# amcolex/ofdm-sync-math

Measured on AMD Instinct MI355X. Metric: complex Msamples/s through S&C metric kernel @ batch=65536; % HBM roofline, higher is better.
Workload: dtype f32 (c64 in, f64 prefix sums); 1 GPU; cfg3 Schmidl-Cox float32 metric+CFO, N=1024 (L=512), cir1, 65536 streams x 1024 c64 per GPU; global_batch=65536, seq_len=1024, L=512, parallelism=stream-shard x1 (no collectives), placement=auto -> contiguous

## Files before the change

ofdm-sync-math_amd/csrc/aa_fast.hip:

```cpp
#include <cfloat>
#include <cmath>
#include "ofs_common.h"
#include "aa_gate.h"
#include "ofdmsync.h"

using namespace ofs;

namespace {

constexpr int FAST_WG = 64;
constexpr int TMAX = 1024;
constexpr int FAST_CAP_LDS = 160 * 1024 / 10;
constexpr int FAST_CAP_LDS_FULL = 23000;

typedef float nf4 __attribute__((ext_vector_type(4)));
typedef float nf2 __attribute__((ext_vector_type(2)));
typedef float pf2 __attribute__((ext_vector_type(2)));
__device__ __forceinline__ pf2 mulc_acc(pf2 c, pf2 d, pf2 acc) {
    acc = __builtin_elementwise_fma(c, d.xx, acc);
    return __builtin_elementwise_fma(c.yx, pf2{d.y, -d.y}, acc);
}
template <int SP>
__device__ __forceinline__ void st_out(float4* p, float4 v) {
    const nf4 d = nf4{v.x, v.y, v.z, v.w};
    if constexpr (SP == 1) __builtin_nontemporal_store(d, reinterpret_cast<nf4*>(p));
    else *p = v;
}
template <int SP>
__device__ __forceinline__ void st_out(float2* p, float2 v) {
    const nf2 d = nf2{v.x, v.y};
    if constexpr (SP == 1) __builtin_nontemporal_store(d, reinterpret_cast<nf2*>(p));
    else *p = v;
}

template <int LP>
__device__ __forceinline__ float4 ld_x(const char* p) {
    if constexpr (LP == 1) {
        const nf4 v = __builtin_nontemporal_load(reinterpret_cast<const nf4*>(p));
        return make_float4(v.x, v.y, v.z, v.w);
    } else {
        return *reinterpret_cast<const float4*>(p);
    }
}

template <int SP>
__device__ __forceinline__ void st_rows2(float* span, const float (&a)[2], const float (&b)[2], int lane) {
    const bool odd = (lane & 1) != 0;
    const int idx = (lane < 32 ? 2 * lane : 2 * lane - 63) * 4;
    float o[4];
#pragma unroll
    for (int e = 0; e < 2; ++e) {
        const int ai = __float_as_int(a[e]), bi = __float_as_int(b[e]);
        const int bdn = dpp_i<0xA0>(bi);
        const int aup = dpp_i<0xF5>(ai);
        const int we = odd ? bdn : ai;
        const int wo = odd ? bi : aup;
        o[e] = __int_as_float(__builtin_amdgcn_ds_bpermute(idx, we));
        o[2 + e] = __int_as_float(__builtin_amdgcn_ds_bpermute(idx, wo));
    }
    st_out<SP>(reinterpret_cast<float4*>(span) + lane, make_float4(o[0], o[1], o[2], o[3]));
}


template <int E, int MR, int NA, bool DO, bool S32, int SV = 0, int FS = 0, int LP = 0>
__global__ __launch_bounds__(FAST_WG) void aa_fast_kernel(AaFastArgs a) {
    static_assert(SV == 0 || (E == 2 && NA == 1 && !DO), "store-path variants: one-antenna E = 2 storing kernel");
    static_assert(FS == 0 || (SV == 3 && !S32), "full-stream form: the headline's kernel");
    static_assert(LP == 0 || FS != 0, "load-policy arms: the full-stream form");
    constexpr bool FULL = FS != 0;
    constexpr int SP = SV & 1;
    constexpr bool RP = (SV & 2) != 0;
    constexpr int RL = 64 * E;
    constexpr int RW = TMAX / RL;
    constexpr int L = MR * RL;
    constexpr int V4 = E / 2;
    static_assert(MR >= 1 && MR <= RW, "window must fit the stream tile");
    const int lane = threadIdx.x & 63;
    const int w = FULL ? 0 : threadIdx.x >> 6;
    const int64_t b = (int64_t)(NA == 1 ? blockIdx.x : xcd_block()) + w;
    if (b >= a.B) return;
    const int T = FULL ? TMAX : (int)a.T;
    const uint32_t lo16 = 16u * (uint32_t)lane;
    float4 xreg[NA][RW][V4];
    if constexpr (FULL) {
        const char* const xb = reinterpret_cast<const char*>(a.x) + b * (TMAX * 8);
#pragma unroll
        for (int k = 0; k < RW; ++k) xreg[0][k][0] = ld_x<LP>(xb + RL * 8 * k + lo16);
    } else {
#pragma unroll
        for (int t = 0; t < NA; ++t) {
            const float2* xs = reinterpret_cast<const float2*>(a.x) + (b * NA + t) * a.T;
#pragma unroll
            for (int k = 0; k < RW; ++k)
#pragma unroll
                for (int j = 0; j < V4; ++j) {
                    int n = RL * k + E * lane + 2 * j;
                    n = n < T ? n : T - 2;
                    xreg[t][k][j] = *reinterpret_cast<const float4*>(xs + n);
                }
        }
    }
    auto xrow = [&](int t, int k, pf2 (&c)[E]) {
#pragma unroll
        for (int j = 0; j < V4; ++j) {
            const bool ok = FULL || RL * k + E * lane + 2 * j < T;
            const float4 v = xreg[t][k][j];
            c[2 * j] = ok ? pf2{v.x, v.y} : pf2{0.f, 0.f};
            c[2 * j + 1] = ok ? pf2{v.z, v.w} : pf2{0.f, 0.f};
        }
    };

    pf2 sS[MR][E];
    float sE[MR][E];
    double Cr[RW + 1], Ci[RW + 1], Ce[RW + 1];
    Cr[0] = Ci[0] = Ce[0] = 0.0;

    AaRowGate<E, float, false, (bool)(DO || NA == 1)> gate;
    const bool detect = FULL || a.detect;
    if (detect)
        gate.init(a.hyst, L, a.thr, a.fs, a.max_ev, a.ev_i + b * (int64_t)a.max_ev * 4,
                  a.ev_r + b * (int64_t)a.max_ev * 4);

    float* Pout = DO ? nullptr : reinterpret_cast<float*>(a.P);
    float* Rout = DO ? nullptr : reinterpret_cast<float*>(a.R);
    float* Mout = DO ? nullptr : reinterpret_cast<float*>(a.M);
    const float floor_ = 1e-6f * (float)L;
    float hR[2] = {0.f, 0.f}, hM[2] = {0.f, 0.f};
    const bool head = !DO && a.head_resident != 0;
    char* const Pb = FULL ? reinterpret_cast<char*>(a.P) + b * (TMAX * 8) : nullptr;
    float* const Rb = FULL ? reinterpret_cast<float*>(a.R) + b * TMAX : nullptr;
    float* const Mb = FULL ? reinterpret_cast<float*>(a.M) + b * TMAX : nullptr;

#pragma unroll
    for (int k = 0; k < RW; ++k) {
        if (FULL || RL * k < T) {
            const int nb = RL * k + E * lane;
            pf2 av[E];
            float aE[E];
#pragma unroll
            for (int e = 0; e < E; ++e) { av[e] = pf2{0.f, 0.f}; aE[e] = 0.f; }
#pragma unroll
            for (int t = 0; t < NA; ++t) {
                pf2 c[E];
                xrow(t, k, c);
// ... 302 lines not shown
        if (p < s.nrows) s.load_row(p, s.nx[p]);
    s.detect = a.detect != 0;
    if (s.detect)
        s.gate.init(a.hyst, S::L, a.thr, a.fs, a.max_ev, a.ev_i + b * (int64_t)a.max_ev * 4,
                    a.ev_r + b * (int64_t)a.max_ev * 4);
    s.Pout = DO ? nullptr : reinterpret_cast<float2*>(a.P);
    s.Rout = DO ? nullptr : reinterpret_cast<float*>(a.R);
    s.Mout = DO ? nullptr : reinterpret_cast<float*>(a.M);
    s.Vout = DO ? nullptr : a.valid;
    s.head = !DO && a.head_resident != 0;
    s.floor_ = 1e-6f * (float)S::L;

    s.template block<true, true>(0);
    int k0 = S::PER;
    for (; k0 + S::PER + S::PD <= s.full_rows; k0 += S::PER) s.template block<false, false>(k0);
    for (; k0 < s.nrows; k0 += S::PER) s.template block<false, true>(k0);
    if (a.detect) s.gate.finish(lane, s.Ti, a.n_ev + b);
}

template <int E, int MR, int NA>
int launch_stream(const AaFastArgs& a, hipStream_t st) {
    const bool det_only = a.detect && !a.P && !a.R && !a.M && !a.valid;
    constexpr int WGD = stream_wg(NA, true), WGS = stream_wg(NA, false);
    const int64_t grid = det_only ? (a.B + WGD / 64 - 1) / (WGD / 64) : (a.B + WGS / 64 - 1) / (WGS / 64);
    using S = AaStream<E, MR, NA, false>;
    constexpr size_t lag_lds = (size_t)(WGS / 64) * (S::LDSLAG ? MR : 1) * NA * S::V4 * 64 * 16;
    constexpr size_t cap_total = 24 * 1024;
    const size_t dflt = (!det_only && NA == 2 && cap_total > lag_lds) ? cap_total - lag_lds : 0;
    const size_t shm = ofs::variant(ofs::V_OCC_LDS) == INT64_MIN ? dflt : ofs::occ_lds();
    if (det_only)
        hipLaunchKernelGGL((aa_stream_kernel<E, MR, NA, true>), dim3((unsigned)grid), dim3(WGD), shm, st, a);
    else
        hipLaunchKernelGGL((aa_stream_kernel<E, MR, NA, false>), dim3((unsigned)grid), dim3(WGS), shm, st, a);
    return hipGetLastError() == hipSuccess ? 1 : OFS_EHIP;
}

template <int E, int NA>
int launch_stream_mr(int mr, const AaFastArgs& a, hipStream_t st) {
    if (mr == 8) return launch_stream<E, 8, NA>(a, st);
    if constexpr (E == 2) {
        switch (mr) {
            case 1: return launch_stream<E, 1, NA>(a, st);
            case 2: return launch_stream<E, 2, NA>(a, st);
            case 4: return launch_stream<E, 4, NA>(a, st);
        }
    }
    return 0;
}

bool scan32(bool det_only) {
    const int64_t v = ofs::variant(det_only ? ofs::V_FAST_SCAN_DO : ofs::V_FAST_SCAN);
    if (v == 32 || v == 64) return v == 32;
    return det_only;
}

float thr_as_f32(double thr) {
    if (thr != thr || thr == (double)INFINITY || thr == -(double)INFINITY) return (float)thr;
    if (thr > (double)FLT_MAX) return INFINITY;
    if (thr < -(double)FLT_MAX) return -FLT_MAX;
    float f = (float)thr;
    if ((double)f < thr) f = nextafterf(f, INFINITY);
    return f;
}

template <int E, int MR, int NA>
int launch(const AaFastArgs& a, hipStream_t st) {
    const bool det_only = a.detect && !a.P && !a.R && !a.M && !a.valid;
    const bool s32 = scan32(det_only);
    const dim3 grid((unsigned)a.B), blk(FAST_WG);
    const int64_t pad = ofs::variant_or(ofs::V_FAST_LDS, (!det_only && NA == 1) ? FAST_CAP_LDS : 0);
    const size_t shm = pad > 0 && pad <= 65536 ? (size_t)pad : 0;
    if constexpr (E == 2 && NA == 1) {
        if (!det_only && !s32) {
            const int sv = (ofs::variant_or(ofs::V_FAST_RMPAIR, 1) != 0 ? 2 : 0) | (ofs::variant_or(ofs::V_FAST_ST_POLICY, 1) == 1 ? 1 : 0);
            if constexpr (MR == 1 || MR == 2 || MR == 4) {
                if (sv == 3 && a.T == TMAX && a.P && a.R && a.M && !a.valid && a.detect && a.n_ev && a.ev_i && a.ev_r &&
                    !ofs::variant_off(ofs::V_FAST_FULL)) {
                    AaFastArgs f = a;
                    f.thr32 = thr_as_f32(a.thr);
                    const int64_t padf = ofs::variant_or(ofs::V_FAST_LDS, FAST_CAP_LDS_FULL);
                    const size_t shmf = padf > 0 && padf <= 65536 ? (size_t)padf : 0;
                    const bool ff = (a.hyst > 1 ? a.hyst : 1) >= 64 * E;
                    const bool nt = ofs::variant(ofs::V_FAST_LD_POLICY) != 0;
                    if (ff && nt) hipLaunchKernelGGL((aa_fast_kernel<E, MR, NA, false, false, 3, 1, 1>), grid, blk, shmf, st, f);
                    else if (ff) hipLaunchKernelGGL((aa_fast_kernel<E, MR, NA, false, false, 3, 1, 0>), grid, blk, shmf, st, f);
                    else if (nt) hipLaunchKernelGGL((aa_fast_kernel<E, MR, NA, false, false, 3, 2, 1>), grid, blk, shmf, st, f);
                    else hipLaunchKernelGGL((aa_fast_kernel<E, MR, NA, false, false, 3, 2, 0>), grid, blk, shmf, st, f);
                    return hipGetLastError() == hipSuccess ? 1 : OFS_EHIP;
                }
            }
            switch (sv) {
                case 0: hipLaunchKernelGGL((aa_fast_kernel<E, MR, NA, false, false, 0>), grid, blk, shm, st, a); break;
                case 1: hipLaunchKernelGGL((aa_fast_kernel<E, MR, NA, false, false, 1>), grid, blk, shm, st, a); break;
                case 2: hipLaunchKernelGGL((aa_fast_kernel<E, MR, NA, false, false, 2>), grid, blk, shm, st, a); break;
                default: hipLaunchKernelGGL((aa_fast_kernel<E, MR, NA, false, false, 3>), grid, blk, shm, st, a);
            }
            return hipGetLastError() == hipSuccess ? 1 : OFS_EHIP;
        }
    }
    if (det_only && s32) hipLaunchKernelGGL((aa_fast_kernel<E, MR, NA, true, true>), grid, blk, shm, st, a);
    else if (det_only) hipLaunchKernelGGL((aa_fast_kernel<E, MR, NA, true, false>), grid, blk, shm, st, a);
    else if (s32) hipLaunchKernelGGL((aa_fast_kernel<E, MR, NA, false, true>), grid, blk, shm, st, a);
    else hipLaunchKernelGGL((aa_fast_kernel<E, MR, NA, false, false>), grid, blk, shm, st, a);
    return hipGetLastError() == hipSuccess ? 1 : OFS_EHIP;
}

template <int E, int NA, int MR = 1>
int launch_mr(int mr, const AaFastArgs& a, hipStream_t st) {
    if constexpr (MR > TMAX / (64 * E)) {
        return 0;
    } else {
        if (mr == MR) return launch<E, MR, NA>(a, st);
        return launch_mr<E, NA, MR + 1>(mr, a, st);
    }
}

template <int NA>
int launch_e(int E, int mr, const AaFastArgs& a, hipStream_t st) {
    switch (E) {
        case 2: return launch_mr<2, NA>(mr, a, st);
        case 4: return launch_mr<4, NA>(mr, a, st);
        case 8: return launch_mr<8, NA>(mr, a, st);
    }
    return 0;
}

int pick_e(int L) {
    const int forced = (int)ofs::variant_or(ofs::V_FAST_E, 0);
    if (forced == 2 || forced == 4 || forced == 8) return (L % (64 * forced) == 0) ? forced : 0;
    for (int e : {2, 4, 8})
        if (L % (64 * e) == 0) return e;
    return 0;
}

int pick_e_do(int L) {
    const int forced = (int)ofs::variant_or(ofs::V_FAST_E_DO, 0);
    for (int e : {forced, 4, 8, 2})
        if ((e == 2 || e == 4 || e == 8) && L % (64 * e) == 0) return e;
    return 0;
}

}

int ofs_aa_fast_plan(int fmt, int precision, int n_ant, int64_t T, int L) {
    if (fmt != OFS_C64 || precision != OFS_FP32) return 0;
    if (n_ant != 1 && n_ant != 2) return 0;
    if (T < 1 || L < 128) return 0;
    if (T <= TMAX && !(T & 1) && L <= TMAX) {
        const int E = pick_e(L);
        if (E) return 10 * E + L / (64 * E);
    }
    if (T > 0x7fffffff - 1024) return 0;
    for (int e : {2, 4}) {
        if (L % (64 * e)) continue;
        const int mr = L / (64 * e);
        if (mr == 1 || mr == 2 || mr == 4 || mr == 8) return 100 + 10 * e + mr;
    }
    return 0;
}

int ofs_aa_fast_try(int fmt, int precision, int n_ant, const AaFastArgs& a, hipStream_t st) {
    const int plan = ofs_aa_fast_plan(fmt, precision, n_ant, a.T, a.L);
    if (!plan) return 0;
    if (plan >= 100) {
        const int E = (plan - 100) / 10, mr = plan % 10;
        if (E == 2) return n_ant == 1 ? launch_stream_mr<2, 1>(mr, a, st) : launch_stream_mr<2, 2>(mr, a, st);
// ... 10 lines not shown
```

ofdm-sync-math_amd/csrc/ofdmsync.hip:

```cpp
#include <hip/hip_runtime.h>
#include <stdint.h>
#include <math.h>
#include "ofdmsync.h"
#include "ofs_common.h"
#include <atomic>
#include <string.h>

namespace {

constexpr int WG = 256;
constexpr int EPT = 4;
constexpr int ROW = 64 * EPT;
constexpr int PASS = WG * EPT;
constexpr int EVBLK = 1024;
constexpr int MAXSLOT = 32;

enum Mode { M_AA = 0, M_SC = 1, M_COMB = 2, M_MINN = 3, M_RTL = 4 };

template <bool EX> struct Prec { using R = float; };
template <> struct Prec<true> { using R = double; };

template <int FMT, class R>
__device__ __forceinline__ void ldx(const void* p, int64_t i, R& re, R& im) {
    if constexpr (FMT == OFS_C64) {
// ... 644 lines not shown
    }
}

constexpr int LEN_MAX_FP32 = 3072;
constexpr int LEN_MAX_FP64 = 3584;

struct Plan { int64_t chunk; int32_t n_chunks, len_max, nrows_max; size_t lds; };

template <class R>
static int make_plan(int64_t T, int64_t n_out, int lo_x, int hi_x, int nq, bool exact, Plan& p) {
    const int halo = hi_x - lo_x;
    const int len_cap = exact ? LEN_MAX_FP64 : LEN_MAX_FP32;
    const int64_t chunk_cap = (int64_t)len_cap - halo;
    if (chunk_cap < 1) return OFS_ETOOLONG;
    int64_t n_chunks = (n_out + chunk_cap - 1) / chunk_cap;
    if (n_chunks < 1) n_chunks = 1;
    int64_t chunk = (n_out + n_chunks - 1) / n_chunks;
    int64_t max_len = chunk + halo;
    if (max_len > T) max_len = T;
    int len_max = (int)((max_len + 3) & ~3ll);
    if (len_max < 4) len_max = 4;
    const int nrows_max = ((len_max + PASS - 1) / PASS) * (PASS / ROW);
    p.chunk = chunk; p.n_chunks = (int32_t)n_chunks; p.len_max = len_max; p.nrows_max = nrows_max;
    p.lds = win_lds_bytes<R>(len_max, nrows_max, nq);
    return OFS_OK;
}

template <int FMT, bool EX, int MODE>
static int launch_win(WinArgs a, int64_t B, const Plan& p, hipStream_t st) {
    auto k = win_kernel<FMT, EX, MODE>;
    if (p.lds > 65536) {
        if (hipFuncSetAttribute((const void*)k, hipFuncAttributeMaxDynamicSharedMemorySize, (int)p.lds) != hipSuccess)
            return OFS_EHIP;
    }
    a.chunk = p.chunk; a.n_chunks = p.n_chunks; a.len_max = p.len_max; a.nrows_max = p.nrows_max;
    const int64_t grid = B * (int64_t)p.n_chunks;
    if (grid > 0x7fffffffll) return OFS_EINVAL;
    hipLaunchKernelGGL(k, dim3((unsigned)grid), dim3(WG), p.lds, st, a);
    return hipGetLastError() == hipSuccess ? OFS_OK : OFS_EHIP;
}

template <int MODE>
static int dispatch_win(int fmt, int precision, WinArgs a, int64_t B, int lo_x, int hi_x,
                        hipStream_t st, Plan* plan_out) {
    constexpr int nq = NQ<MODE>::v;
    Plan p;
    int rc;
    const bool ex = precision == OFS_FP64;
    rc = ex ? make_plan<double>(a.T, a.n_out, lo_x, hi_x, nq, true, p)
            : make_plan<float>(a.T, a.n_out, lo_x, hi_x, nq, false, p);
    if (rc) return rc;
    if (plan_out) *plan_out = p;
    a.lo_x = lo_x; a.hi_x = hi_x;
    if (ex) {
        switch (fmt) {
            case OFS_C64: return launch_win<OFS_C64, true, MODE>(a, B, p, st);
            case OFS_C128: return launch_win<OFS_C128, true, MODE>(a, B, p, st);
            case OFS_CI16: return launch_win<OFS_CI16, true, MODE>(a, B, p, st);
        }
    } else if constexpr (MODE != M_RTL) {
        switch (fmt) {
            case OFS_C64: return launch_win<OFS_C64, false, MODE>(a, B, p, st);
            case OFS_C128: return launch_win<OFS_C128, false, MODE>(a, B, p, st);
            case OFS_CI16: return launch_win<OFS_CI16, false, MODE>(a, B, p, st);
        }
    }
    return OFS_EINVAL;
}

static bool fmt_ok(int f) { return f == OFS_C64 || f == OFS_C128 || f == OFS_CI16; }
static bool prec_ok(int p) { return p == OFS_FP32 || p == OFS_FP64; }

}

extern "C" {

int32_t ofs_version(void) { return 100; }


static const char* const kVariantNames[ofs::V_COUNT] = {
    "EXACT", "FAST_E", "FAST_E_DO", "FAST_SCAN", "FAST_SCAN_DO", "RTL_WPB", "PARK_DIRECT", "ZW64",
    "ZW64_GRID", "ZS", "ZF_ITEMS", "ZS_PAIR", "ZS_DEFER", "ZS_BPL", "ZS_C", "ZS_GBLK", "MC_FUSED",
    "MC_FUSE_X", "ZC_SEQ", "ZC_NODMA", "BE_FAST", "MC_PERS", "FAST_LDS", "OCC_LDS",
    "FAST_RMPAIR", "FAST_ST_POLICY", "FAST_HEAD", "FAST_FULL", "FAST_LD_POLICY"};
struct VariantTable {
    int64_t v[ofs::V_COUNT];
    VariantTable() { for (auto& x : v) x = OFS_VARIANT_UNSET; }
};
static thread_local VariantTable g_variants;

static int variant_index(const char* name) {
    if (!name) return -1;
    for (int i = 0; i < ofs::V_COUNT; ++i)
        if (strcmp(name, kVariantNames[i]) == 0) return i;
    return -1;
}

int32_t ofs_debug_reset_variants(void) {
    for (auto& x : g_variants.v) x = OFS_VARIANT_UNSET;
    return OFS_OK;
}

int32_t ofs_debug_set_variant(const char* name, int64_t value) {
    const int i = variant_index(name);
    if (i < 0) return OFS_EINVAL;
    g_variants.v[i] = value;
    return OFS_OK;
}

int64_t ofs_debug_get_variant(const char* name) {
    const int i = variant_index(name);
    return i < 0 ? OFS_VARIANT_UNSET : ofs::variant((ofs::Variant)i);
}

const char* ofs_status_string(int32_t s) {
    switch (s) {
        case OFS_OK: return "ok";
        case OFS_EINVAL: return "invalid argument";
        case OFS_ETOOLONG: return "window/halo does not fit one LDS tile";
        case OFS_EHIP: return "HIP launch error";
        case OFS_ESHORT: return "stream shorter than one symbol";
        case OFS_EFFT: return "rocFFT error";
        default: return "unknown status";
    }
}

int32_t ofs_aa_detect(int32_t in_fmt, const void* x, int64_t B, int32_t n_ant, int64_t T,
                      int32_t L, int32_t precision, void* P, void* R, void* M, uint8_t* valid,
                      int32_t detect, double threshold, int32_t hysteresis, double sample_rate,
                      int32_t max_events, int32_t* n_events, int64_t* ev_int, double* ev_real,
                      void* stream) {
    return ofs_aa_detect_ex(in_fmt, x, B, n_ant, T, L, precision, P, R, M, valid, detect, threshold, hysteresis,
                            sample_rate, max_events, n_events, ev_int, ev_real, stream, 0u);
}

int32_t ofs_aa_detect_ex(int32_t in_fmt, const void* x, int64_t B, int32_t n_ant, int64_t T,
                         int32_t L, int32_t precision, void* P, void* R, void* M, uint8_t* valid,
                         int32_t detect, double threshold, int32_t hysteresis, double sample_rate,
                         int32_t max_events, int32_t* n_events, int64_t* ev_int, double* ev_real,
                         void* stream, uint32_t flags) {
    if (flags & ~(uint32_t)OFS_AA_HEAD_RESIDENT) return OFS_EINVAL;
    if (!(fmt_ok(in_fmt) || in_fmt == OFS_CP12) || !prec_ok(precision) || OFS_MISSING(x, B * T) || B < 0 || n_ant < 1 ||
        T < 0 || L < 1)
        return OFS_EINVAL;
    if (detect && (OFS_MISSING(n_events, B) || max_events < 0 ||
                   (max_events > 0 && B > 0 && (!ev_int || !ev_real))))
        return OFS_EINVAL;
    if (B == 0 || T == 0) return OFS_OK;
    hipStream_t st = (hipStream_t)stream;
    {
        AaFastArgs f{};
        f.x = x; f.B = B; f.T = T; f.L = L; f.P = P; f.R = R; f.M = M; f.valid = valid;
        f.detect = detect; f.thr = threshold; f.hyst = hysteresis; f.fs = sample_rate;
        f.max_ev = max_events; f.n_ev = n_events; f.ev_i = ev_int; f.ev_r = ev_real;
        f.head_resident = (flags & OFS_AA_HEAD_RESIDENT) != 0 && !ofs::variant_off(ofs::V_FAST_HEAD);
        int frc = ofs_aa_fast_try(in_fmt, precision, n_ant, f, st);
        if (frc == 1) return OFS_OK;
        if (frc < 0) return frc;
        frc = ofs_aa_exact_try(in_fmt, precision, n_ant, f, st);
        if (frc == 1) return OFS_OK;
        if (frc < 0) return frc;
    }
    if (in_fmt == OFS_CP12) return OFS_EINVAL;
    WinArgs a{};
    a.x = x; a.T = T; a.n_out = T; a.nb = n_ant; a.D = L; a.W = L;
    a.P = P; a.R = R; a.M = M; a.valid = valid;
    a.detect = detect; a.thr = threshold; a.hyst = hysteresis; a.fs = sample_rate;
// ... 205 lines not shown
```

ofdm-sync-math_amd/csrc/ofs_common.h:

```cpp
#pragma once
#include <hip/hip_runtime.h>
#include <stdint.h>

#define OFS_MISSING(p, n) ((p) == nullptr && (int64_t)(n) > 0)

namespace ofs {

enum Variant : int {
    V_EXACT, V_FAST_E, V_FAST_E_DO, V_FAST_SCAN, V_FAST_SCAN_DO, V_RTL_WPB, V_PARK_DIRECT, V_ZW64,
    V_ZW64_GRID, V_ZS, V_ZF_ITEMS, V_ZS_PAIR, V_ZS_DEFER, V_ZS_BPL, V_ZS_C, V_ZS_GBLK, V_MC_FUSED,
    V_MC_FUSE_X, V_ZC_SEQ, V_ZC_NODMA, V_BE_FAST, V_MC_PERS, V_FAST_LDS, V_OCC_LDS,
    V_FAST_RMPAIR, V_FAST_ST_POLICY, V_FAST_HEAD, V_FAST_FULL, V_FAST_LD_POLICY, V_COUNT
};
int64_t variant(Variant v);
inline bool variant_is(Variant v, int64_t value) { return variant(v) == value; }
inline bool variant_off(Variant v) { return variant(v) == 0; }
inline bool variant_on(Variant v) { const int64_t x = variant(v); return x != INT64_MIN && x != 0; }
inline int64_t variant_or(Variant v, int64_t dflt) { const int64_t x = variant(v); return x == INT64_MIN ? dflt : x; }
inline size_t occ_lds() { const int64_t x = variant(V_OCC_LDS); return x > 0 && x <= 65536 ? (size_t)x : 0; }


template <int CTRL>
__device__ __forceinline__ int dpp_i(int v) {
    return __builtin_amdgcn_mov_dpp(v, CTRL, 0xf, 0xf, false);
}
template <int CTRL>
__device__ __forceinline__ double dpp_d(double v) {
    const int lo = dpp_i<CTRL>(__double2loint(v));
    const int hi = dpp_i<CTRL>(__double2hiint(v));
    return __hiloint2double(hi, lo);
}

__device__ __forceinline__ double wave_scan_add(double v, int lane) {
    const int rl = lane & 15;
    double t;
    t = dpp_d<0x111>(v); if (rl >= 1) v += t;
    t = dpp_d<0x112>(v); if (rl >= 2) v += t;
    t = dpp_d<0x114>(v); if (rl >= 4) v += t;
    t = dpp_d<0x118>(v); if (rl >= 8) v += t;
    t = dpp_d<0x142>(v); if ((lane & 31) >= 16) v += t;
    t = dpp_d<0x143>(v); if (lane >= 32) v += t;
    return v;
}

__device__ __forceinline__ int wave_scan_max(int v, int lane) {
    const int rl = lane & 15;
    int t;
    t = dpp_i<0x111>(v); if (rl >= 1) v = max(v, t);
    t = dpp_i<0x112>(v); if (rl >= 2) v = max(v, t);
    t = dpp_i<0x114>(v); if (rl >= 4) v = max(v, t);
    t = dpp_i<0x118>(v); if (rl >= 8) v = max(v, t);
    t = dpp_i<0x142>(v); if ((lane & 31) >= 16) v = max(v, t);
    t = dpp_i<0x143>(v); if (lane >= 32) v = max(v, t);
    return v;
}

__device__ __forceinline__ double wave_shr1(double v, int lane, double first) {
    const double t = dpp_d<0x138>(v);
    return lane == 0 ? first : t;
}
__device__ __forceinline__ int wave_shr1(int v, int lane, int first) {
    const int t = dpp_i<0x138>(v);
    return lane == 0 ? first : t;
}

__device__ __forceinline__ double readlane(double v, int j) {
    const int lo = __builtin_amdgcn_readlane(__double2loint(v), j);
    const int hi = __builtin_amdgcn_readlane(__double2hiint(v), j);
    return __hiloint2double(hi, lo);
}
__device__ __forceinline__ float readlane(float v, int j) {
    return __int_as_float(__builtin_amdgcn_readlane(__float_as_int(v), j));
}
__device__ __forceinline__ int readlane(int v, int j) { return __builtin_amdgcn_readlane(v, j); }

template <int CTRL, int RMASK = 0xf>
__device__ __forceinline__ int dpp_old(int old, int v) {
    return __builtin_amdgcn_update_dpp(old, v, CTRL, RMASK, 0xf, false);
}
template <class Op>
__device__ __forceinline__ int dpp_reduce_bits(int v, int ident, Op op) {
    v = op(v, dpp_old<0x111>(ident, v));
    v = op(v, dpp_old<0x112>(ident, v));
    v = op(v, dpp_old<0x114>(ident, v));
    v = op(v, dpp_old<0x118>(ident, v));
    v = op(v, dpp_old<0x142, 0xa>(ident, v));
    v = op(v, dpp_old<0x143, 0xc>(ident, v));
    return __builtin_amdgcn_readlane(v, 63);
}
__device__ __forceinline__ float wave_max(float v) {
    const int r = dpp_reduce_bits(__float_as_int(v), __float_as_int(-__builtin_huge_valf()), [](int a, int b) {
        return __float_as_int(fmaxf(__int_as_float(a), __int_as_float(b)));
    });
    return __int_as_float(r);
}
// ... 32 lines not shown
    return blockIdx.x;
#endif
}

__device__ __forceinline__ float fast_atan2f(float y, float x) {
    const float ax = fabsf(x), ay = fabsf(y);
    const float mx = fmaxf(ax, ay), mn = fminf(ax, ay);
    const float a = mx > 0.f ? mn * __builtin_amdgcn_rcpf(mx) : 0.f;
    const float s = a * a;
    float r = -0.004054530523717403f;
    r = fmaf(r, s, 0.02186284027993679f);
    r = fmaf(r, s, -0.055912185460329056f);
    r = fmaf(r, s, 0.09642189741134644f);
    r = fmaf(r, s, -0.1390862762928009f);
    r = fmaf(r, s, 0.19946566224098206f);
    r = fmaf(r, s, -0.33329859375953674f);
    r = fmaf(r, s, 0.9999993443489075f);
    r *= a;
    if (ay > ax) r = 1.5707963267948966f - r;
    if (x < 0.f) r = 3.141592653589793f - r;
    return __builtin_copysignf(r, y);
}

template <int CTRL, int RMASK = 0xf>
__device__ __forceinline__ double dppz(double v) {
    const int lo = __builtin_amdgcn_update_dpp(0, __double2loint(v), CTRL, RMASK, 0xf, true);
    const int hi = __builtin_amdgcn_update_dpp(0, __double2hiint(v), CTRL, RMASK, 0xf, true);
    return __hiloint2double(hi, lo);
}
__device__ __forceinline__ double scan_add(double v) {
    v += dppz<0x111>(v);
    v += dppz<0x112>(v);
    v += dppz<0x114>(v);
    v += dppz<0x118>(v);
    v += dppz<0x142, 0xa>(v);
    v += dppz<0x143, 0xc>(v);
    return v;
}
__device__ __forceinline__ double shr1z(double v) { return dppz<0x138>(v); }

template <int CTRL, int RMASK = 0xf>
__device__ __forceinline__ int dppz_i(int v) {
    return __builtin_amdgcn_update_dpp(0, v, CTRL, RMASK, 0xf, true);
}
__device__ __forceinline__ int scan_add_i32(int v) {
    v += dppz_i<0x111>(v);
    v += dppz_i<0x112>(v);
    v += dppz_i<0x114>(v);
    v += dppz_i<0x118>(v);
    v += dppz_i<0x142, 0xa>(v);
    v += dppz_i<0x143, 0xc>(v);
    return v;
}

template <int CTRL, int RMASK = 0xf>
__device__ __forceinline__ float dppz_f(float v) {
    return __int_as_float(__builtin_amdgcn_update_dpp(0, __float_as_int(v), CTRL, RMASK, 0xf, true));
}
__device__ __forceinline__ float scan_add_f32(float v) {
    v += dppz_f<0x111>(v);
    v += dppz_f<0x112>(v);
    v += dppz_f<0x114>(v);
    v += dppz_f<0x118>(v);
    v += dppz_f<0x142, 0xa>(v);
    v += dppz_f<0x143, 0xc>(v);
    return v;
}

struct RowScan { float x, u; double tot; };
template <bool F32>
__device__ __forceinline__ RowScan row_scan(float v) {
    if constexpr (F32) {
        const float i = scan_add_f32(v);
        const float t = readlane(i, 63);
        return RowScan{dppz_f<0x138>(i), t - i, (double)t};
    } else {
        const double i = scan_add((double)v);
        const double t = readlane(i, 63);
        return RowScan{(float)shr1z(i), (float)(t - i), t};
    }
}


__device__ __forceinline__ void lds_dma16(const void* g, const void* lds) {
    const uint32_t m = (uint32_t)(uintptr_t)(__attribute__((address_space(3))) const void*)lds;
    asm volatile("s_mov_b32 m0, %1\n\ts_nop 0\n\tglobal_load_lds_dwordx4 %0, off" ::"v"(g), "s"(m) : "memory", "m0");
}


#define OFS_VMW(i) case i: asm volatile("s_waitcnt vmcnt(" #i ")" ::: "memory"); break;
__device__ __forceinline__ void vmcnt_wait(int n) {
    switch (n < 63 ? n : 63) {
        OFS_VMW(0) OFS_VMW(1) OFS_VMW(2) OFS_VMW(3) OFS_VMW(4) OFS_VMW(5) OFS_VMW(6) OFS_VMW(7)
        OFS_VMW(8) OFS_VMW(9) OFS_VMW(10) OFS_VMW(11) OFS_VMW(12) OFS_VMW(13) OFS_VMW(14) OFS_VMW(15)
        OFS_VMW(16) OFS_VMW(17) OFS_VMW(18) OFS_VMW(19) OFS_VMW(20) OFS_VMW(21) OFS_VMW(22) OFS_VMW(23)
        OFS_VMW(24) OFS_VMW(25) OFS_VMW(26) OFS_VMW(27) OFS_VMW(28) OFS_VMW(29) OFS_VMW(30) OFS_VMW(31)
        OFS_VMW(32) OFS_VMW(33) OFS_VMW(34) OFS_VMW(35) OFS_VMW(36) OFS_VMW(37) OFS_VMW(38) OFS_VMW(39)
        OFS_VMW(40) OFS_VMW(41) OFS_VMW(42) OFS_VMW(43) OFS_VMW(44) OFS_VMW(45) OFS_VMW(46) OFS_VMW(47)
        OFS_VMW(48) OFS_VMW(49) OFS_VMW(50) OFS_VMW(51) OFS_VMW(52) OFS_VMW(53) OFS_VMW(54) OFS_VMW(55)
        OFS_VMW(56) OFS_VMW(57) OFS_VMW(58) OFS_VMW(59) OFS_VMW(60) OFS_VMW(61) OFS_VMW(62)
        default: asm volatile("s_waitcnt vmcnt(63)" ::: "memory"); break;
    }
}
#undef OFS_VMW

}

struct AaFastArgs {
    const void* x;
    int64_t B, T;
    int32_t L;
    void* P; void* R; void* M; uint8_t* valid;
    int32_t detect; double thr; int32_t hyst; double fs;
    int32_t max_ev; int32_t* n_ev; int64_t* ev_i; double* ev_r;
    int32_t head_resident;
    float thr32;
};
int ofs_aa_fast_try(int fmt, int precision, int n_ant, const AaFastArgs& a, hipStream_t st);
int ofs_aa_fast_plan(int fmt, int precision, int n_ant, int64_t T, int L);

int ofs_aa_exact_plan(int fmt, int precision, int n_ant, int64_t T, int L);
int ofs_aa_exact_try(int fmt, int precision, int n_ant, const AaFastArgs& a, hipStream_t st);
struct RtlExactCall {
    const void* x; int64_t B, T; int32_t Q;
    int32_t shift, smooth_mode, frac_bits; double thr_value;
    double* corr_total; double* corr_positive; double* smooth; double* energy_total;
    double* corr_scaled; double* energy_scaled; uint8_t* mvalid; uint8_t* above;
    int32_t detect, hyst, toff, max_ev; int32_t* n_ev; int64_t* ev; int64_t* open_start;
};
int ofs_rtl_exact_plan(int fmt, int n_br, int64_t T, int Q);
int ofs_rtl_exact_try(int fmt, int n_br, const RtlExactCall& c, hipStream_t st);

struct WinFastArgs {
    const void* x; int64_t B, T; int N;
    void* M; void* P; void* R;
};
int ofs_win_fast_try(int mode, int fmt, int precision, int n_br, const WinFastArgs& a, hipStream_t st);
int ofs_win_fast_plan(int mode, int fmt, int precision, int n_br, int64_t T, int N);
int ofs_sc_minn_fast_plan(int fmt, int precision, int n_br, int64_t T, int N);
int ofs_sc_minn_fast_try(int fmt, int precision, int n_br, const void* x, int64_t B, int64_t T, int N,
                         void* Ms, void* Ps, void* Rs, void* Mm, void* Pm, void* Rm, hipStream_t st);
```

Measured before the change: 359,800 Msamples/s.

## Add lean full-stream Schmidl-Cox kernel with register-resident input and batched DPP scans

Adds a specialised one-antenna, full-stream metric kernel that loads the whole 1024-sample stream into registers up front, interleaves three row scans (energy, real and imaginary correlation) with DPP row broadcasts that keep their registers, and delays R/M stores by one row pair. It becomes the default path for the headline configuration unless FAST_LEAN is turned off. The aim is to cut instruction count and scan latency relative to the general templated kernel and to hide load latency by issuing every load early. In exchange it uses more VGPRs for the register tile and carries a second copy of the kernel logic that has to stay in sync with the original.

```diff
diff --git a/ofdm-sync-math_amd/csrc/aa_fast.hip b/ofdm-sync-math_amd/csrc/aa_fast.hip
--- a/ofdm-sync-math_amd/csrc/aa_fast.hip
+++ b/ofdm-sync-math_amd/csrc/aa_fast.hip
@@ -2,64 +2,17 @@
 #include <cmath>
 #include "ofs_common.h"
 #include "aa_gate.h"
+#include "aa_fast_io.h"
 #include "ofdmsync.h"
 
 using namespace ofs;
 
+int ofs_aa_lean_launch(int mr, bool ff, bool nt, bool head, unsigned grid, size_t shm, hipStream_t st, const AaFastArgs& f);
+
 namespace {
 
-constexpr int FAST_WG = 64;
-constexpr int TMAX = 1024;
 constexpr int FAST_CAP_LDS = 160 * 1024 / 10;
 constexpr int FAST_CAP_LDS_FULL = 23000;
-
-typedef float nf4 __attribute__((ext_vector_type(4)));
-typedef float nf2 __attribute__((ext_vector_type(2)));
-typedef float pf2 __attribute__((ext_vector_type(2)));
-__device__ __forceinline__ pf2 mulc_acc(pf2 c, pf2 d, pf2 acc) {
-    acc = __builtin_elementwise_fma(c, d.xx, acc);
-    return __builtin_elementwise_fma(c.yx, pf2{d.y, -d.y}, acc);
-}
-template <int SP>
-__device__ __forceinline__ void st_out(float4* p, float4 v) {
-    const nf4 d = nf4{v.x, v.y, v.z, v.w};
-    if constexpr (SP == 1) __builtin_nontemporal_store(d, reinterpret_cast<nf4*>(p));
-    else *p = v;
-}
-template <int SP>
-__device__ __forceinline__ void st_out(float2* p, float2 v) {
-    const nf2 d = nf2{v.x, v.y};
-    if constexpr (SP == 1) __builtin_nontemporal_store(d, reinterpret_cast<nf2*>(p));
-    else *p = v;
-}
-
-template <int LP>
-__device__ __forceinline__ float4 ld_x(const char* p) {
-    if constexpr (LP == 1) {
-        const nf4 v = __builtin_nontemporal_load(reinterpret_cast<const nf4*>(p));
-        return make_float4(v.x, v.y, v.z, v.w);
-    } else {
-        return *reinterpret_cast<const float4*>(p);
-    }
-}
-
-template <int SP>
-__device__ __forceinline__ void st_rows2(float* span, const float (&a)[2], const float (&b)[2], int lane) {
-    const bool odd = (lane & 1) != 0;
-    const int idx = (lane < 32 ? 2 * lane : 2 * lane - 63) * 4;
-    float o[4];
-#pragma unroll
-    for (int e = 0; e < 2; ++e) {
-        const int ai = __float_as_int(a[e]), bi = __float_as_int(b[e]);
-        const int bdn = dpp_i<0xA0>(bi);
-        const int aup = dpp_i<0xF5>(ai);
-        const int we = odd ? bdn : ai;
-        const int wo = odd ? bi : aup;
-        o[e] = __int_as_float(__builtin_amdgcn_ds_bpermute(idx, we));
-        o[2 + e] = __int_as_float(__builtin_amdgcn_ds_bpermute(idx, wo));
-    }
-    st_out<SP>(reinterpret_cast<float4*>(span) + lane, make_float4(o[0], o[1], o[2], o[3]));
-}
 
 
 template <int E, int MR, int NA, bool DO, bool S32, int SV = 0, int FS = 0, int LP = 0>
@@ -528,6 +481,8 @@
                     const size_t shmf = padf > 0 && padf <= 65536 ? (size_t)padf : 0;
                     const bool ff = (a.hyst > 1 ? a.hyst : 1) >= 64 * E;
                     const bool nt = ofs::variant(ofs::V_FAST_LD_POLICY) != 0;
+                    if (!ofs::variant_off(ofs::V_FAST_LEAN))
+                        return ofs_aa_lean_launch(MR, ff, nt, a.head_resident != 0, (unsigned)a.B, shmf, st, f);
                     if (ff && nt) hipLaunchKernelGGL((aa_fast_kernel<E, MR, NA, false, false, 3, 1, 1>), grid, blk, shmf, st, f);
                     else if (ff) hipLaunchKernelGGL((aa_fast_kernel<E, MR, NA, false, false, 3, 1, 0>), grid, blk, shmf, st, f);
                     else if (nt) hipLaunchKernelGGL((aa_fast_kernel<E, MR, NA, false, false, 3, 2, 1>), grid, blk, shmf, st, f);
diff --git a/ofdm-sync-math_amd/csrc/aa_fast_io.h b/ofdm-sync-math_amd/csrc/aa_fast_io.h
--- /dev/null
+++ b/ofdm-sync-math_amd/csrc/aa_fast_io.h
@@ -0,0 +1,57 @@
+#pragma once
+#include "ofs_common.h"
+
+namespace {
+using ofs::dpp_i;
+
+constexpr int FAST_WG = 64;
+constexpr int TMAX = 1024;
+typedef float nf4 __attribute__((ext_vector_type(4)));
+typedef float nf2 __attribute__((ext_vector_type(2)));
+typedef float pf2 __attribute__((ext_vector_type(2)));
+__device__ __forceinline__ pf2 mulc_acc(pf2 c, pf2 d, pf2 acc) {
+    acc = __builtin_elementwise_fma(c, d.xx, acc);
+    return __builtin_elementwise_fma(c.yx, pf2{d.y, -d.y}, acc);
+}
+template <int SP>
+__device__ __forceinline__ void st_out(float4* p, float4 v) {
+    const nf4 d = nf4{v.x, v.y, v.z, v.w};
+    if constexpr (SP == 1) __builtin_nontemporal_store(d, reinterpret_cast<nf4*>(p));
+    else *p = v;
+}
+template <int SP>
+__device__ __forceinline__ void st_out(float2* p, float2 v) {
+    const nf2 d = nf2{v.x, v.y};
+    if constexpr (SP == 1) __builtin_nontemporal_store(d, reinterpret_cast<nf2*>(p));
+    else *p = v;
+}
+
+template <int LP>
+__device__ __forceinline__ float4 ld_x(const char* p) {
+    if constexpr (LP == 1) {
+        const nf4 v = __builtin_nontemporal_load(reinterpret_cast<const nf4*>(p));
+        return make_float4(v.x, v.y, v.z, v.w);
+    } else {
+        return *reinterpret_cast<const float4*>(p);
+    }
+}
+
+template <int SP>
+__device__ __forceinline__ void st_rows2(float* span, const float (&a)[2], const float (&b)[2], int lane) {
+    const bool odd = (lane & 1) != 0;
+    const int idx = (lane < 32 ? 2 * lane : 2 * lane - 63) * 4;
+    float o[4];
+#pragma unroll
+    for (int e = 0; e < 2; ++e) {
+        const int ai = __float_as_int(a[e]), bi = __float_as_int(b[e]);
+        const int bdn = dpp_i<0xA0>(bi);
+        const int aup = dpp_i<0xF5>(ai);
+        const int we = odd ? bdn : ai;
+        const int wo = odd ? bi : aup;
+        o[e] = __int_as_float(__builtin_amdgcn_ds_bpermute(idx, we));
+        o[2 + e] = __int_as_float(__builtin_amdgcn_ds_bpermute(idx, wo));
+    }
+    st_out<SP>(reinterpret_cast<float4*>(span) + lane, make_float4(o[0], o[1], o[2], o[3]));
+}
+
+}
diff --git a/ofdm-sync-math_amd/csrc/aa_lean.hip b/ofdm-sync-math_amd/csrc/aa_lean.hip
--- /dev/null
+++ b/ofdm-sync-math_amd/csrc/aa_lean.hip
@@ -0,0 +1,176 @@
+#include "ofs_common.h"
+#include "aa_gate.h"
+#include "aa_fast_io.h"
+#include "ofdmsync.h"
+
+using namespace ofs;
+
+namespace {
+
+__device__ __forceinline__ float4 shuf_rows2(const float (&a)[2], const float (&b)[2], int lane) {
+    const bool odd = (lane & 1) != 0;
+    const int idx = (lane < 32 ? 2 * lane : 2 * lane - 63) * 4;
+    float o[4];
+#pragma unroll
+    for (int e = 0; e < 2; ++e) {
+        const int ai = __float_as_int(a[e]), bi = __float_as_int(b[e]);
+        const int bdn = dpp_i<0xA0>(bi);
+        const int aup = dpp_i<0xF5>(ai);
+        const int we = odd ? bdn : ai;
+        const int wo = odd ? bi : aup;
+        o[e] = __int_as_float(__builtin_amdgcn_ds_bpermute(idx, we));
+        o[2 + e] = __int_as_float(__builtin_amdgcn_ds_bpermute(idx, wo));
+    }
+    return make_float4(o[0], o[1], o[2], o[3]);
+}
+
+template <int MR, int FS, int LP, bool HD>
+__global__ __launch_bounds__(FAST_WG) void aa_lean_kernel(AaFastArgs a) {
+    constexpr int E = 2, SP = 1;
+    constexpr int RL = 64 * E;
+    constexpr int RW = TMAX / RL;
+    constexpr int L = MR * RL;
+    static_assert(MR >= 1 && MR <= RW - 2, "the last row pair lies behind the window");
+    const int lane = threadIdx.x & 63;
+    const int64_t b = (int64_t)blockIdx.x;
+    if (b >= a.B) return;
+    constexpr int T = TMAX;
+    const uint32_t lo16 = 16u * (uint32_t)lane;
+    float4 xreg[RW];
+    const char* const xb = reinterpret_cast<const char*>(a.x) + b * (TMAX * 8);
+#pragma unroll
+    for (int k = 0; k < RW; ++k) xreg[k] = ld_x<LP>(xb + RL * 8 * k + lo16);
+    auto xrow = [&](int k, pf2 (&c)[E]) {
+        const float4 v = xreg[k];
+        c[0] = pf2{v.x, v.y};
+        c[1] = pf2{v.z, v.w};
+    };
+
+    pf2 sS[MR][E];
+    float sE[MR][E];
+    double Cr[RW + 1], Ci[RW + 1], Ce[RW + 1];
+    Cr[0] = Ci[0] = Ce[0] = 0.0;
+
+    AaRowGate<E, float, false, true> gate;
+    gate.init(a.hyst, L, a.thr, a.fs, a.max_ev, a.ev_i + b * (int64_t)a.max_ev * 4, a.ev_r + b * (int64_t)a.max_ev * 4);
+
+    const float floor_ = 1e-6f * (float)L;
+    float hR[2] = {0.f, 0.f}, hM[2] = {0.f, 0.f};
+    constexpr bool head = HD;
+    ScanKeep zk[3];
+    float4 oR = make_float4(0.f, 0.f, 0.f, 0.f), oM = oR;
+    char* const Pb = reinterpret_cast<char*>(a.P) + b * (TMAX * 8);
+    float* const Rb = reinterpret_cast<float*>(a.R) + b * TMAX;
+    float* const Mb = reinterpret_cast<float*>(a.M) + b * TMAX;
+
+#pragma unroll
+    for (int k = 0; k < RW; ++k) {
+        const int nb = RL * k + E * lane;
+        pf2 av[E];
+        float aE[E];
+#pragma unroll
+        for (int e = 0; e < E; ++e) { av[e] = pf2{0.f, 0.f}; aE[e] = 0.f; }
+        {
+            pf2 c[E];
+            xrow(k, c);
+#pragma unroll
+            for (int e = 0; e < E; ++e) aE[e] += fmaf(c[e].x, c[e].x, c[e].y * c[e].y);
+            if (k >= MR) {
+                pf2 d[E];
+                xrow(k - MR, d);
+#pragma unroll
+                for (int e = 0; e < E; ++e) av[e] = mulc_acc(c[e], d[e], av[e]);
+            }
+        }
+        pf2 fS[E], gS[E];
+        float fE[E], gE[E];
+        fS[0] = av[0]; fE[0] = aE[0];
+#pragma unroll
+        for (int e = 1; e < E; ++e) { fS[e] = fS[e - 1] + av[e]; fE[e] = fE[e - 1] + aE[e]; }
+        gS[E - 1] = pf2{0.f, 0.f}; gE[E - 1] = 0.f;
+#pragma unroll
+        for (int e = E - 2; e >= 0; --e) { gS[e] = gS[e + 1] + av[e + 1]; gE[e] = gE[e + 1] + aE[e + 1]; }
+        RowScan sEr, sRr{0.f, 0.f, 0.0}, sIr{0.f, 0.f, 0.0};
+        if (k >= MR) {
+            const float v3[3] = {fE[E - 1], fS[E - 1].x, fS[E - 1].y};
+            RowScan r3[3];
+            row_scan_keep3(v3, zk, r3);
+            sEr = r3[0]; sRr = r3[1]; sIr = r3[2];
+        } else {
+            sEr = row_scan_keep(fE[E - 1], zk[0]);
+        }
+        if (k >= 2 && (k & 1) == 0) {
+            st_out<SP>(reinterpret_cast<float4*>(Rb + RL * (k - 2)) + lane, oR);
+            if (!(k - 1 < MR && head)) st_out<SP>(reinterpret_cast<float4*>(Mb + RL * (k - 2)) + lane, oM);
+        }
+        const double totR = sRr.tot, totI = sIr.tot, totE = sEr.tot;
+        const pf2 xS = pf2{sRr.x, sIr.x};
+        const float xE = sEr.x;
+        const pf2 uS = pf2{sRr.u, sIr.u};
+        const float uE = sEr.u;
+        Cr[k + 1] = Cr[k] + totR; Ci[k + 1] = Ci[k] + totI; Ce[k + 1] = Ce[k] + totE;
+        const pf2 wS = pf2{(float)((k >= MR) ? (Cr[k] - Cr[k - MR + 1]) : Cr[k]),
+                           (float)((k >= MR) ? (Ci[k] - Ci[k - MR + 1]) : Ci[k])};
+        const float wE = (float)((k >= MR) ? (Ce[k] - Ce[k - MR + 1]) : Ce[k]);
+
+        float pf[E][2], mf[E], pmf[E], rf[E];
+#pragma unroll
+        for (int e = 0; e < E; ++e) {
+            pf2 P = wS + (xS + fS[e]);
+            float RR = wE + (xE + fE[e]);
+            if (k >= MR) { P += sS[k % MR][e]; RR += sE[k % MR][e]; }
+            sS[k % MR][e] = uS + gS[e]; sE[k % MR][e] = uE + gE[e];
+            const float pm = fmaf(P.x, P.x, P.y * P.y);
+            float m = 0.f;
+            if (k >= MR && RR > floor_) m = fminf(pm * __builtin_amdgcn_rcpf(RR * RR), 1.f);
+            pf[e][0] = P.x; pf[e][1] = P.y; rf[e] = RR; mf[e] = m; pmf[e] = pm;
+        }
+
+        const bool pm_row = !(k < MR && head);
+        if (pm_row) st_out<SP>(reinterpret_cast<float4*>(Pb + RL * 8 * k + lo16), make_float4(pf[0][0], pf[0][1], pf[1][0], pf[1][1]));
+        if ((k & 1) == 0) {
+            hR[0] = rf[0]; hR[1] = rf[1]; hM[0] = mf[0]; hM[1] = mf[1];
+        } else {
+            oR = shuf_rows2(hR, rf, lane);
+            if (pm_row) oM = shuf_rows2(hM, mf, lane);
+        }
+
+        if (k >= MR) {
+            float pr[E], pi[E];
+#pragma unroll
+            for (int e = 0; e < E; ++e) { pr[e] = pf[e][0]; pi[e] = pf[e][1]; }
+            bool ab[E];
+#pragma unroll
+            for (int e = 0; e < E; ++e) ab[e] = mf[e] >= a.thr32;
+            gate.template row_flags<FS, true>(lane, k, nb, T, ab, pmf, pr, pi, mf);
+        }
+    }
+    st_out<SP>(reinterpret_cast<float4*>(Rb + RL * (RW - 2)) + lane, oR);
+    st_out<SP>(reinterpret_cast<float4*>(Mb + RL * (RW - 2)) + lane, oM);
+    gate.finish(lane, T, a.n_ev + b);
+}
+
+template <int MR>
+int launch_lean(bool ff, bool nt, bool head, dim3 grid, dim3 blk, size_t shm, hipStream_t st, const AaFastArgs& f) {
+#define OFS_LEAN(FS_, LP_) \
+    do { if (head) hipLaunchKernelGGL((aa_lean_kernel<MR, FS_, LP_, true>), grid, blk, shm, st, f); \
+         else hipLaunchKernelGGL((aa_lean_kernel<MR, FS_, LP_, false>), grid, blk, shm, st, f); } while (0)
+    if (ff && nt) OFS_LEAN(1, 1);
+    else if (ff) OFS_LEAN(1, 0);
+    else if (nt) OFS_LEAN(2, 1);
+    else OFS_LEAN(2, 0);
+#undef OFS_LEAN
+    return hipGetLastError() == hipSuccess ? 1 : OFS_EHIP;
+}
+
+}
+
+int ofs_aa_lean_launch(int mr, bool ff, bool nt, bool head, unsigned grid, size_t shm, hipStream_t st, const AaFastArgs& f) {
+    const dim3 g(grid), blk(FAST_WG);
+    switch (mr) {
+        case 1: return launch_lean<1>(ff, nt, head, g, blk, shm, st, f);
+        case 2: return launch_lean<2>(ff, nt, head, g, blk, shm, st, f);
+        case 4: return launch_lean<4>(ff, nt, head, g, blk, shm, st, f);
+    }
+    return 0;
+}
diff --git a/ofdm-sync-math_amd/csrc/ofdmsync.hip b/ofdm-sync-math_amd/csrc/ofdmsync.hip
--- a/ofdm-sync-math_amd/csrc/ofdmsync.hip
+++ b/ofdm-sync-math_amd/csrc/ofdmsync.hip
@@ -750,7 +750,7 @@
     "EXACT", "FAST_E", "FAST_E_DO", "FAST_SCAN", "FAST_SCAN_DO", "RTL_WPB", "PARK_DIRECT", "ZW64",
     "ZW64_GRID", "ZS", "ZF_ITEMS", "ZS_PAIR", "ZS_DEFER", "ZS_BPL", "ZS_C", "ZS_GBLK", "MC_FUSED",
     "MC_FUSE_X", "ZC_SEQ", "ZC_NODMA", "BE_FAST", "MC_PERS", "FAST_LDS", "OCC_LDS",
-    "FAST_RMPAIR", "FAST_ST_POLICY", "FAST_HEAD", "FAST_FULL", "FAST_LD_POLICY"};
+    "FAST_RMPAIR", "FAST_ST_POLICY", "FAST_HEAD", "FAST_FULL", "FAST_LD_POLICY", "FAST_LEAN"};
 struct VariantTable {
     int64_t v[ofs::V_COUNT];
     VariantTable() { for (auto& x : v) x = OFS_VARIANT_UNSET; }
diff --git a/ofdm-sync-math_amd/csrc/ofs_common.h b/ofdm-sync-math_amd/csrc/ofs_common.h
--- a/ofdm-sync-math_amd/csrc/ofs_common.h
+++ b/ofdm-sync-math_amd/csrc/ofs_common.h
@@ -10,7 +10,7 @@
     V_EXACT, V_FAST_E, V_FAST_E_DO, V_FAST_SCAN, V_FAST_SCAN_DO, V_RTL_WPB, V_PARK_DIRECT, V_ZW64,
     V_ZW64_GRID, V_ZS, V_ZF_ITEMS, V_ZS_PAIR, V_ZS_DEFER, V_ZS_BPL, V_ZS_C, V_ZS_GBLK, V_MC_FUSED,
     V_MC_FUSE_X, V_ZC_SEQ, V_ZC_NODMA, V_BE_FAST, V_MC_PERS, V_FAST_LDS, V_OCC_LDS,
-    V_FAST_RMPAIR, V_FAST_ST_POLICY, V_FAST_HEAD, V_FAST_FULL, V_FAST_LD_POLICY, V_COUNT
+    V_FAST_RMPAIR, V_FAST_ST_POLICY, V_FAST_HEAD, V_FAST_FULL, V_FAST_LD_POLICY, V_FAST_LEAN, V_COUNT
 };
 int64_t variant(Variant v);
 inline bool variant_is(Variant v, int64_t value) { return variant(v) == value; }
@@ -209,6 +209,56 @@
 }
 
 
+struct ScanKeep { int l15 = 0, h15 = 0, l31 = 0, h31 = 0; };
+template <int CTRL, int RMASK>
+__device__ __forceinline__ double dpp_keep(double v, int& lo, int& hi) {
+    lo = __builtin_amdgcn_update_dpp(lo, __double2loint(v), CTRL, RMASK, 0xf, true);
+    hi = __builtin_amdgcn_update_dpp(hi, __double2hiint(v), CTRL, RMASK, 0xf, true);
+    return __hiloint2double(hi, lo);
+}
+__device__ __forceinline__ RowScan row_scan_keep(float v, ScanKeep& z) {
+    double i = (double)v;
+    i += dppz<0x111>(i);
+    i += dppz<0x112>(i);
+    i += dppz<0x114>(i);
+    i += dppz<0x118>(i);
+    i += dpp_keep<0x142, 0xa>(i, z.l15, z.h15);
+    i += dpp_keep<0x143, 0xc>(i, z.l31, z.h31);
+    const double t = readlane(i, 63);
+    return RowScan{dppz_f<0x138>((float)i), (float)(t - i), t};
+}
+template <int CTRL>
+__device__ __forceinline__ void scan_step3(double (&i)[3]) {
+    double t[3];
+#pragma unroll
+    for (int j = 0; j < 3; ++j) t[j] = dppz<CTRL>(i[j]);
+#pragma unroll
+    for (int j = 0; j < 3; ++j) i[j] += t[j];
+}
+__device__ __forceinline__ void row_scan_keep3(const float (&v)[3], ScanKeep (&z)[3], RowScan (&r)[3]) {
+    double i[3], t[3];
+#pragma unroll
+    for (int j = 0; j < 3; ++j) i[j] = (double)v[j];
+    scan_step3<0x111>(i);
+    scan_step3<0x112>(i);
+    scan_step3<0x114>(i);
+    scan_step3<0x118>(i);
+#pragma unroll
+    for (int j = 0; j < 3; ++j) t[j] = dpp_keep<0x142, 0xa>(i[j], z[j].l15, z[j].h15);
+#pragma unroll
+    for (int j = 0; j < 3; ++j) i[j] += t[j];
+#pragma unroll
+    for (int j = 0; j < 3; ++j) t[j] = dpp_keep<0x143, 0xc>(i[j], z[j].l31, z[j].h31);
+#pragma unroll
+    for (int j = 0; j < 3; ++j) i[j] += t[j];
+#pragma unroll
+    for (int j = 0; j < 3; ++j) {
+        const double tot = readlane(i[j], 63);
+        r[j] = RowScan{dppz_f<0x138>((float)i[j]), (float)(tot - i[j]), tot};
+    }
+}
+
+
 __device__ __forceinline__ void lds_dma16(const void* g, const void* lds) {
     const uint32_t m = (uint32_t)(uintptr_t)(__attribute__((address_space(3))) const void*)lds;
     asm volatile("s_mov_b32 m0, %1\n\ts_nop 0\n\tglobal_load_lds_dwordx4 %0, off" ::"v"(g), "s"(m) : "memory", "m0");
```

Result: no change. 359,300 Msamples/s (-0.1%).
